# exoclime/HELIOS

Measured on AMD Instinct MI355X. Metric: rad-conv iterations/sec x (lambda-bins x layers), higher is better.
Workload: dtype f64; 1 GPU; BASELINE config 2: single column, 10 000 bins x 100 layers, premixed corr-k, isotropic scattering; nbin=10000, nlayer=100, ny=20, species=0, columns_per_gpu=1, columns_total=1, loop=radiative, parallelism=columns sharded, 1 per GPU

## Files before the change

helios_amd/csrc/rt_flux_kernel.inc:

```
template <int ROWS, int K = 0, bool MATRIX = false>
HX_FLUX_HEAD {
    using CT = HX_PLANE_T;
    extern __shared__ __align__(16) double smem[];
    const int col = a.reverse ? (int)(gridDim.y - 1 - blockIdx.y) : (int)blockIdx.y;
    if (a.done[col]) return;
    const int bx = a.reverse ? (int)(gridDim.x - 1 - blockIdx.x) : (int)blockIdx.x;
    const bool keep_state_cached = (int)(blockIdx.y * gridDim.x + blockIdx.x) >= a.cache_state_from;
    const int NN = a.H + 3, I = a.I;
    double* sB = smem;
    double* acc = sB + (size_t)a.nxb * NN;
    double* stage = acc + (size_t)a.nxb * 2 * I;
    const hx_rt_column cp = a.colpar[col];
    const size_t nc = (size_t)a.Y * a.X;
    const int k = K ? K : a.k;

    for (int t = threadIdx.x; t < a.nxb * NN; t += blockDim.x) {
        const int xl = t / NN, n = t - xl * NN, x = bx * a.nxb + xl;
        sB[t] = x < a.X ? a.Bn[((size_t)col * a.X + x) * NN + n] : 0.0;
    }
    for (int t = threadIdx.x; t < a.nxb * 2 * I; t += blockDim.x) acc[t] = 0.0;
    __syncthreads();

    for (int part = 0; part < a.nparts; part++) {
        const LaneMap m = lane_map(a, bx, part, opaque_tid());
        const size_t toff = m.tile * (size_t)ROWS * 64 + m.lane;
        const CT* ctile = HX_PLANES + col * a.coef_col + m.tile * (size_t)a.nplane * ROWS * 64 + m.lane;
        double* utile = a.Utile + col * a.flux_col + toff;
        double al[ROWS], be[ROWS], sd[ROWS], su[ROWS], Uo[ROWS], Do[ROWS];
#pragma unroll
        for (int r = 0; r < ROWS; r++) {
            al[r] = __builtin_nontemporal_load(ctile + (0 * ROWS + r) * 64);
            be[r] = __builtin_nontemporal_load(ctile + (1 * ROWS + r) * 64);
            sd[r] = __builtin_nontemporal_load(ctile + (2 * ROWS + r) * 64);
            if (!MATRIX) Uo[r] = __builtin_nontemporal_load(utile + r * 64);
        }
        if constexpr (sizeof(CT) == sizeof(double)) {
            if (a.has_vp) {
#pragma unroll
                for (int r = 0; r < ROWS; r++) su[r] = __builtin_nontemporal_load(ctile + (a.pl_vp * ROWS + r) * 64);
            } else {
#pragma unroll
                for (int r = 0; r < ROWS; r++) su[r] = a.Kconst * ((1.0 - al[r]) - be[r]) - sd[r];
            }
        } else {
            if (a.has_vp) {
#pragma unroll
                for (int r = 0; r < ROWS; r++) su[r] = __builtin_nontemporal_load(ctile + (a.pl_vp * ROWS + r) * 64);
            }
#pragma unroll
            for (int r = 0; r < ROWS; r++) {
                const double rest = plane_decode(al[r], be[r]);
                su[r] = (a.has_vp ? su[r] : a.Kconst * rest) - sd[r];
            }
        }
        double U0 = 0.0, boaK = 0.0, Fdir0 = 0.0, albedo = 0.0;
        if (m.valid && m.j == 0) {
            if (!MATRIX) U0 = a.U0[col * nc + m.sp];
            boaK = a.boaK[col * nc + m.sp];
            Fdir0 = a.Fdir0[col * nc + m.sp];
            albedo = a.surf_albedo[(size_t)col * a.X + m.x];
        }
        const double w = m.valid ? 0.5 * a.gauss_w[m.y] : 0.0;
        const double* Bx = sB + (size_t)(m.valid ? m.xl : 0) * NN;
#pragma unroll
        for (int r = 0; r < ROWS; r++) {
            const int h = min(m.j * ROWS + r, a.H - 1);
            const double Bb = Bx[h], Bt = a.iso ? Bb : Bx[h + 1], upc = sd[r], vpc = su[r];
            sd[r] = upc * Bb + vpc * Bt;
            su[r] = upc * Bt + vpc * Bb;
        }
        if (a.dir_beam == 1) {
            constexpr int BEAM_GROUP = ROWS <= 8 ? ROWS : HX_BEAM_GROUP;
#pragma unroll
            for (int r0 = 0; r0 < ROWS; r0 += BEAM_GROUP) {
                double bd[BEAM_GROUP], bu[BEAM_GROUP];
#pragma unroll
                for (int u = 0; u < BEAM_GROUP; u++)
                    if (r0 + u < ROWS) {
                        bd[u] = __builtin_nontemporal_load(ctile + (a.pl_dd * ROWS + r0 + u) * 64);
                        bu[u] = __builtin_nontemporal_load(ctile + ((a.pl_dd + 1) * ROWS + r0 + u) * 64);
                    }
                __builtin_amdgcn_sched_barrier(0);
#pragma unroll
                for (int u = 0; u < BEAM_GROUP; u++)
                    if (r0 + u < ROWS) {
                        sd[r0 + u] += bd[u];
                        su[r0 + u] += bu[u];
                    }
                __builtin_amdgcn_sched_barrier(0);
            }
        }
        const double rs = cp.R_star / cp.a;
        const double D_toa = (1.0 - a.dir_beam) * cp.f_factor * (rs * rs) * HX_PI * Bx[a.H + 1];
        const double B_surf = Bx[a.H + 2];

        const bool odd0 = (m.j * ROWS) & 1;
        const double thr_even = (a.iso || odd0) ? 1e-100 : 0.0, thr_odd = (a.iso || !odd0) ? 1e-100 : 0.0;
        if constexpr (MATRIX) {
            const bool scatters = m.valid ? a.trigger[col * nc + m.sp] != 0 : false;
            const bool flip_negative = scatters && !a.iso;
            const double tiny_d = scatters ? 0.0 : 1e-100;
            const double tiny_u_even = scatters ? 0.0 : ((a.iso || odd0) ? 1e-100 : 0.0), tiny_u_odd = scatters ? 0.0 : ((a.iso || !odd0) ? 1e-100 : 0.0);
            auto patch = [&](double v, double tiny) { return flip_negative ? (v < 1e-100 ? fabs(v) : v) : tiny_abs_below(v, tiny); };
            Moebius P = {1.0, 0.0, 0.0, 1.0};
#pragma unroll
            for (int r = 0; r < ROWS; r++) {
                const double omb = 1.0 - be[r];
                const double m11 = fma(al[r], al[r], be[r] * omb), m12 = (omb - al[r]) * (omb + al[r]);
                const double n11 = fma(m11, P.p11, m12 * P.p21), n12 = fma(m11, P.p12, m12 * P.p22);
                P.p21 = fma(be[r], P.p11, omb * P.p21);
                P.p22 = fma(be[r], P.p12, omb * P.p22);
                P.p11 = n11;
                P.p12 = n12;
            }
            {
                const double sc = 1.0 / fmax(fmax(fabs(P.p11), fabs(P.p12)), fmax(fabs(P.p21), fabs(P.p22)));
                P.p11 *= sc; P.p12 *= sc; P.p21 *= sc; P.p22 *= sc;
            }
            moebius_scan_up<K>(P, m.j, k);
            double e11 = K ? below_fixed<K>(P.p11) : from_lane_below<1>(P.p11, k), e12 = K ? below_fixed<K>(P.p12) : from_lane_below<1>(P.p12, k);
            double e21 = K ? below_fixed<K>(P.p21) : from_lane_below<1>(P.p21, k), e22 = K ? below_fixed<K>(P.p22) : from_lane_below<1>(P.p22, k);
            const double alb = K ? group_first_lane<K>(albedo, m.lane) : __shfl(albedo, 0, k);
            double rho = 1.0 - fma(e11, 1.0 - alb, e12) / fma(e21, 1.0 - alb, e22);
            if (m.j == 0) rho = alb;
#pragma unroll
            for (int r = 0; r < ROWS; r++) {
                const double inv = HX_MATRIX_RCP(1.0 - be[r] * rho), aa = al[r] * inv;
                su[r] = fma(aa * rho, sd[r], su[r]);
                rho = fma(aa * al[r], rho, be[r]);
                Uo[r] = rho;
                be[r] *= inv;
                sd[r] *= inv;
                al[r] = aa;
            }
            double sigma0 = 0.0;
            if (m.j == 0) sigma0 = albedo * Fdir0 + (1.0 - albedo) * HX_PI * boaK * B_surf;
            sigma0 = K ? group_first_lane<K>(sigma0, m.lane) : __shfl(sigma0, 0, k);
            {
                double A = 1.0, Bc = 0.0;
#pragma unroll
                for (int r = 0; r < ROWS; r++) {
                    Bc = fma(al[r], Bc, su[r]);
                    A *= al[r];
                }
                if (K) {
                    scan_up_fixed<K>(A, Bc, m.j);
                } else if (k == 32) {
                    scan32_up(A, Bc, m.j);
                } else {
                    scan_step_up<1>(A, Bc, m.j, k);
                    scan_step_up<2>(A, Bc, m.j, k);
                    scan_step_up<4>(A, Bc, m.j, k);
                    scan_step_up<8>(A, Bc, m.j, k);
                    scan_step_up<16>(A, Bc, m.j, k);
                    scan_step_up<32>(A, Bc, m.j, k);
                }
                double sg = K ? below_fixed<K>(fma(A, sigma0, Bc)) : from_lane_below<1>(fma(A, sigma0, Bc), k);
                if (m.j == 0) sg = sigma0;
#pragma unroll
                for (int r = 0; r < ROWS; r++) {
                    sd[r] = fma(be[r], sg, sd[r]);
                    sg = fma(al[r], sg, su[r]);
                    su[r] = sg;
                }
            }
            {
                double A = 1.0, Bc = 0.0;
#pragma unroll
                for (int r = ROWS - 1; r >= 0; r--) {
                    Bc = fma(al[r], Bc, sd[r]);
                    A *= al[r];
                }
                if (K) {
                    scan_down_fixed<K>(A, Bc, m.j, m.lane);
                } else if (k == 32) {
                    scan32_down(A, Bc, m.j, m.lane);
                } else {
                    scan_step_down<1>(A, Bc, m.j, k);
                    scan_step_down<2>(A, Bc, m.j, k);
                    scan_step_down<4>(A, Bc, m.j, k);
                    scan_step_down<8>(A, Bc, m.j, k);
                    scan_step_down<16>(A, Bc, m.j, k);
                    scan_step_down<32>(A, Bc, m.j, k);
                }
                double D = K ? above_fixed<K>(fma(A, D_toa, Bc)) : from_lane_above<1>(fma(A, D_toa, Bc), k);
                if (m.j == k - 1) D = D_toa;
#pragma unroll
                for (int r = ROWS - 1; r >= 0; r--) {
                    Uo[r] = patch(fma(Uo[r], D, su[r]), (r & 1) ? tiny_u_odd : tiny_u_even);
                    D = patch(fma(al[r], D, sd[r]), tiny_d);
                    Do[r] = D;
                }
            }
            if (m.j == 0) U0 = patch(fma(albedo, Do[0], sigma0), 0.0);
        } else
        for (int sweep = 0; sweep < a.nsweep; sweep++) {
            {
                double Ubelow = K ? below_fixed<K>(Uo[ROWS - 1]) : from_lane_below<1>(Uo[ROWS - 1], k);
                if (m.j == 0) Ubelow = U0;
                double A = 1.0, Bc = 0.0;
#pragma unroll
                for (int r = ROWS - 1; r >= 0; r--) {
                    const double Uh = r > 0 ? Uo[r - 1] : Ubelow;
                    const double t = fma(be[r], Uh, sd[r]);
                    Bc = fma(al[r], Bc, t);
                    A *= al[r];
                }
                if (K) {
                    scan_down_fixed<K>(A, Bc, m.j, m.lane);
                } else if (k == 32) {
                    scan32_down(A, Bc, m.j, m.lane);
                } else {
                    scan_step_down<1>(A, Bc, m.j, k);
                    scan_step_down<2>(A, Bc, m.j, k);
                    scan_step_down<4>(A, Bc, m.j, k);
                    scan_step_down<8>(A, Bc, m.j, k);
                    scan_step_down<16>(A, Bc, m.j, k);
                    scan_step_down<32>(A, Bc, m.j, k);
                }
                double Din = K ? above_fixed<K>(fma(A, D_toa, Bc)) : from_lane_above<1>(fma(A, D_toa, Bc), k);
                if (m.j == k - 1) Din = D_toa;
                double D = Din;
#pragma unroll
                for (int r = ROWS - 1; r >= 0; r--) {
                    const double Uh = r > 0 ? Uo[r - 1] : Ubelow;
                    D = tiny_abs(fma(al[r], D, fma(be[r], Uh, sd[r])));
                    Do[r] = D;
                }
            }
            if (m.j == 0) U0 = albedo * (Fdir0 + Do[0]) + (1.0 - albedo) * HX_PI * boaK * B_surf;
            const double Ubc = K ? group_first_lane<K>(U0, m.lane) : __shfl(U0, 0, k);
            {
                double Dabove = K ? above_fixed<K>(Do[0]) : from_lane_above<1>(Do[0], k);
                if (m.j == k - 1) Dabove = D_toa;
                double A = 1.0, Bc = 0.0;
#pragma unroll
                for (int r = 0; r < ROWS; r++) {
                    const double Dh = r < ROWS - 1 ? Do[r + 1] : Dabove;
                    const double t = fma(be[r], Dh, su[r]);
                    Bc = fma(al[r], Bc, t);
                    A *= al[r];
                }
                if (K) {
                    scan_up_fixed<K>(A, Bc, m.j);
                } else if (k == 32) {
                    scan32_up(A, Bc, m.j);
                } else {
                    scan_step_up<1>(A, Bc, m.j, k);
                    scan_step_up<2>(A, Bc, m.j, k);
                    scan_step_up<4>(A, Bc, m.j, k);
                    scan_step_up<8>(A, Bc, m.j, k);
                    scan_step_up<16>(A, Bc, m.j, k);
                    scan_step_up<32>(A, Bc, m.j, k);
                }
                double Uin = K ? below_fixed<K>(fma(A, Ubc, Bc)) : from_lane_below<1>(fma(A, Ubc, Bc), k);
                if (m.j == 0) Uin = Ubc;
                double U = Uin;
#pragma unroll
                for (int r = 0; r < ROWS; r++) {
                    const double Dh = r < ROWS - 1 ? Do[r + 1] : Dabove;
                    U = fma(al[r], U, fma(be[r], Dh, su[r]));
                    if (K) U = tiny_abs_below(U, (r & 1) ? thr_odd : thr_even);
                    else if (a.iso || ((m.j * ROWS + r) & 1)) U = tiny_abs(U);
                    Uo[r] = U;
                }
            }
        }

        const LaneMap e = lane_map(a, bx, part, opaque_tid());
#ifdef HX_PROFILING
        const int debug_skip = a.debug_skip;
#else
        constexpr int debug_skip = 0;
#endif
        auto store_state = [&]() {
            const size_t eoff = e.tile * (size_t)ROWS * 64 + e.lane;
            if (!(debug_skip & 2) && (!MATRIX || a.keep_up)) {
                double* ut = a.Utile + col * a.flux_col + eoff;
#pragma unroll
                for (int r = 0; r < ROWS; r++) {
                    if (keep_state_cached) __hip_atomic_store(ut + r * 64, Uo[r], __ATOMIC_RELAXED, __HIP_MEMORY_SCOPE_AGENT);
                    else __builtin_nontemporal_store(Uo[r], ut + r * 64);
                }
            }
            if (a.keep_down) {
                double* dtile = a.Dtile + col * a.flux_col + eoff;
#pragma unroll
                for (int r = 0; r < ROWS; r++) __builtin_nontemporal_store(Do[r], dtile + r * 64);
            }
            if (e.valid && e.j == 0) a.U0[col * nc + e.sp] = U0;
        };
        if (!(debug_skip & 1)) {
            if (e.valid) {
                const int h0 = e.j * ROWS, nrow = a.H - h0;
                double* st = stage + ((size_t)e.yl * a.nxb + e.xl) * 2 * I;
                if (a.iso) {
                    double *pd = st + h0, *pu = st + I + h0 + 1;
#pragma unroll
                    for (int r = 0; r < ROWS; r++)
                        if (r < nrow) {
                            pd[r] = w * Do[r];
                            pu[r] = w * Uo[r];
                        }
                } else {
                    const bool p = h0 & 1;
                    const int q = (h0 + (p ? 1 : 0)) >> 1;
                    double* pe = st + q + (p ? I : 0);
                    double* po = st + q + (p ? -1 : I);
#pragma unroll
                    for (int r = 0; r < ROWS; r++)
                        if (r < nrow) {
                            if ((r & 1) == 0) pe[r >> 1] = w * (p ? Uo[r] : Do[r]);
                            else po[(r + 1) >> 1] = w * (p ? Do[r] : Uo[r]);
                        }
                }
                if (e.j == 0) st[I + 0] = w * U0;
                if (h0 <= a.H - 1 && a.H - 1 < h0 + ROWS) st[a.L] = w * D_toa;
            }
            __syncthreads();
            for (int t = threadIdx.x; t < a.nxb * 2 * I; t += blockDim.x) {
                const int xl = t / (2 * I), rest = t - xl * 2 * I;
                double s = acc[t];
                for (int yl = 0; yl < a.ypb; yl++) s += stage[((size_t)yl * a.nxb + xl) * 2 * I + rest];
                acc[t] = s;
            }
            __syncthreads();
        }
        store_state();
    }
    for (int t = threadIdx.x; t < a.nxb * 2 * I; t += blockDim.x) {
        const int xl = t / (2 * I), rest = t - xl * 2 * I, x = bx * a.nxb + xl;
        if (x >= a.X) continue;
        const int dir = rest / I, i = rest - dir * I;
        (dir == 0 ? a.F_down_band_n : a.F_up_band_n)[((size_t)col * a.X + x) * I + i] = acc[t];
    }
}
```

helios_amd/csrc/rt_kernels.h:

```cpp
#pragma once
#include "rt_fused.h"
#include "conv_adjust.h"
#include "temp_step.h"
#include "two_stream.h"
#include "plane_code.h"

namespace hx {

struct KArgs {
    int X, Y, L, I, H, C;
    int k, ROWS, S, nxb, ypb, nparts, G, NW, nblk_x, nblk, nplane, nchunk, coef_nbx;
    int cloud_lds;
    int scat, dir_beam, clouds, scat_corr, nsweep, keep_down, real_star;
    int iso;
    int has_vp, pl_vp, pl_dd;
    int matrix;
    int* trigger;
    double Kconst;
    int dim, step;
    double epsi, epsi2, g_0, i2s, w_0_limit, w_0_scat_limit, dtau_limit;
    const hx_rt_column* colpar;
    const double *T_lay, *p_lay, *p_int, *dcol_u, *dcol_l, *surf_albedo, *Bstar, *planck_grid;
    const double *opac_wg_lay, *opac_wg_int, *scat_cross_lay, *scat_cross_int, *mmm_lay, *mmm_int;
    const double *cl_abs_lay, *cl_abs_int, *cl_sc_lay, *cl_sc_int, *g0_tot_lay, *g0_tot_int;
    double *half_ray, *half_g0, *half_cab, *half_csc;
    const double *F_dir_wg, *Fc_dir_wg, *F_dir_band_n, *gauss_w, *deltawave;
    double *T_int, *Bn, *coef, *Utile, *Dtile, *U0, *boaK, *Fdir0;
    double *dtau_u, *dtau_l;
    double *F_down_band_n, *F_up_band_n, *tot_part, *F_up_tot, *F_down_tot, *F_net;
    size_t coef_col, flux_col;
    const int* done;
    const TableSet* coltab;
    const double *ktemp, *kpress;
    const TPIndex *tp_lay, *tp_int;
    int ntemp, npress, from_table;
    unsigned long long* diag;
    int* iter_dev;
};

struct FluxArgs {
    int X, Y, L, I, H;
    int k, nxb, ypb, nparts, G, NW;
    int dir_beam, nsweep, keep_down, has_vp, pl_vp, pl_dd, nplane, iso, debug_skip;
    int keep_up;
    int reverse;
    int cache_state_from;
    const int* trigger;
    double Kconst;
    const hx_rt_column* colpar;
    const double *Bn, *coef, *U0_in, *boaK, *Fdir0, *surf_albedo, *gauss_w;
    double *Utile, *Dtile, *U0, *F_down_band_n, *F_up_band_n;
    size_t coef_col, flux_col;
    const int* done;
};

__device__ __forceinline__ double interface_T(const double* T, int i, int L) {
    if (i == 0) return T[0] - 0.5 * (T[1] - T[0]);
    if (i == L) return T[L - 1] + 0.5 * (T[L - 1] - T[L - 2]);
    return T[i - 1] + 0.5 * (T[i] - T[i - 1]);
}

__host__ __device__ __forceinline__ size_t plane_off(int r, int lane, int ROWS) {
    (void)ROWS;
    return (size_t)r * 64 + lane;
}

#ifndef HX_PLANE_KERNELS_ONLY
__global__ void __launch_bounds__(256) k_rt_nodes(KArgs a) {
    __shared__ double tile[32][33];
    const int col = blockIdx.z;
    if (blockIdx.x == 0 && blockIdx.y == 0 && blockIdx.z == 0 && threadIdx.x == 0 && a.iter_dev != nullptr) {
        const int cur = a.iter_dev[0];
        a.iter_dev[1] = cur;
        a.iter_dev[0] = cur + 1;
    }
    if (a.done[col]) return;
    const int NN = a.H + 3;
    const double* T = a.T_lay + (size_t)col * (a.L + 1);
    const int x0 = blockIdx.x * 32, n0 = blockIdx.y * 32;
    const int tx = threadIdx.x & 31, ty = threadIdx.x >> 5;
    if (blockIdx.x == 0 && blockIdx.y == 0)
        for (int i = threadIdx.x; i < a.I; i += blockDim.x)
            a.T_int[(size_t)col * a.I + i] = interface_T(T, i, a.L);
    enum { DEAD, STAR, LEVEL, INT_BOTTOM, INT_TOP, INT_MID };
    const int x = x0 + tx, xc = min(x, a.X - 1);
    int kind[4];
    double Ta[4], Tb[4], star[4];
#pragma unroll
    for (int q = 0; q < 4; q++) {
        const int n = n0 + ty + 8 * q, i = n >> 1;
        int kd, ia, ib = 0;
        if (!(n < NN && x < a.X)) { kd = DEAD; ia = 0; }
        else if (n == a.H + 1) { kd = STAR; ia = 0; }
        else if (n == a.H + 2) { kd = LEVEL; ia = a.L; }
        else if (a.iso) { kd = LEVEL; ia = min(n, a.L - 1); }
        else if (n & 1) { kd = LEVEL; ia = (n - 1) >> 1; }
        else if (i == 0) { kd = INT_BOTTOM; ia = 0; ib = 1; }
        else if (i == a.L) { kd = INT_TOP; ia = a.L - 1; ib = max(a.L - 2, 0); }
        else { kd = INT_MID; ia = i - 1; ib = i; }
        kind[q] = kd;
        Ta[q] = T[ia];
        Tb[q] = T[ib];
        star[q] = kd == STAR ? a.Bstar[(size_t)col * a.X + x] : 0.0;
    }
    int tdown[4], tup[4];
    double tt[4], gd[4], gu[4];
#pragma unroll
    for (int q = 0; q < 4; q++) {
        double Tn = Ta[q];
        if (kind[q] == INT_BOTTOM) Tn = Ta[q] - 0.5 * (Tb[q] - Ta[q]);
        else if (kind[q] == INT_TOP) Tn = Ta[q] + 0.5 * (Ta[q] - Tb[q]);
        else if (kind[q] == INT_MID) Tn = Ta[q] + 0.5 * (Tb[q] - Ta[q]);
        double t = (Tn - 1.0) / a.step;
        t = dmax(0.001, dmin(a.dim - 1.001, t));
        tt[q] = t;
        tdown[q] = (int)floor(t);
        tup[q] = (int)ceil(t);
        gd[q] = a.planck_grid[xc + (size_t)tdown[q] * a.X];
        gu[q] = a.planck_grid[xc + (size_t)tup[q] * a.X];
    }
#pragma unroll
    for (int q = 0; q < 4; q++) {
        double v = gd[q];
        if (tdown[q] != tup[q]) v = gd[q] * (tup[q] - tt[q]) + gu[q] * (tt[q] - tdown[q]);
        if (kind[q] == STAR) v = star[q];
        if (kind[q] != DEAD) tile[ty + 8 * q][tx] = v;
    }
    __syncthreads();
    for (int r = ty; r < 32; r += 8) {
        const int x = x0 + r, n = n0 + tx;
        if (n < NN && x < a.X) a.Bn[((size_t)col * a.X + x) * NN + n] = tile[tx][r];
    }
}

#endif
template <int CTRL, int ROW_MASK>
__device__ __forceinline__ double dpp_move(double v) {
    int lo = __double2loint(v), hi = __double2hiint(v);
    lo = __builtin_amdgcn_update_dpp(lo, lo, CTRL, ROW_MASK, 0xf, false);
    hi = __builtin_amdgcn_update_dpp(hi, hi, CTRL, ROW_MASK, 0xf, false);
    return __hiloint2double(hi, lo);
}

template <int N>
__device__ __forceinline__ double from_lane_below(double v, int k) {
    if (N == 1 && k == 32) return dpp_move<0x138, 0xf>(v);
    if (N < 16 && k <= 16) {
        int lo = __double2loint(v), hi = __double2hiint(v);
        lo = __builtin_amdgcn_update_dpp(lo, lo, 0x110 + (N & 15), 0xf, 0xf, false);
        hi = __builtin_amdgcn_update_dpp(hi, hi, 0x110 + (N & 15), 0xf, 0xf, false);
        return __hiloint2double(hi, lo);
    } else {
        return __shfl_up(v, N);
    }
}
template <int N>
__device__ __forceinline__ double from_lane_above(double v, int k) {
    if (N == 1 && k == 32) return dpp_move<0x130, 0xf>(v);
    if (N < 16 && k <= 16) {
        int lo = __double2loint(v), hi = __double2hiint(v);
        lo = __builtin_amdgcn_update_dpp(lo, lo, 0x100 + (N & 15), 0xf, 0xf, false);
        hi = __builtin_amdgcn_update_dpp(hi, hi, 0x100 + (N & 15), 0xf, 0xf, false);
        return __hiloint2double(hi, lo);
    } else {
        return __shfl_down(v, N);
    }
}

template <int N>
__device__ __forceinline__ void scan_step_down(double& A, double& Bc, int j, int k) {
    if (N < k) {
        const double A2 = from_lane_above<N>(A, k), B2 = from_lane_above<N>(Bc, k);
        if (j + N < k) {
            Bc = fma(A, B2, Bc);
            A *= A2;
        }
    }
}
template <int N>
__device__ __forceinline__ void scan_step_up(double& A, double& Bc, int j, int k) {
    if (N < k) {
        const double A2 = from_lane_below<N>(A, k), B2 = from_lane_below<N>(Bc, k);
        if (j >= N) {
            Bc = fma(A, B2, Bc);
            A *= A2;
        }
    }
}

__device__ __forceinline__ double group_lane16(double v, int lane) {
    const int lo = __double2loint(v), hi = __double2hiint(v);
    const int lo_a = __builtin_amdgcn_readlane(lo, 16), lo_b = __builtin_amdgcn_readlane(lo, 48);
    const int hi_a = __builtin_amdgcn_readlane(hi, 16), hi_b = __builtin_amdgcn_readlane(hi, 48);
    return __hiloint2double(lane < 32 ? hi_a : hi_b, lane < 32 ? lo_a : lo_b);
}

#define HX_SCAN32_ROW_STEP(CTRL, COND)                                              \
    {                                                                               \
        const double A2 = dpp_move<CTRL, 0xf>(A), B2 = dpp_move<CTRL, 0xf>(Bc);     \
        if (COND) {                                                                 \
            Bc = fma(A, B2, Bc);                                                    \
            A *= A2;                                                                \
        }                                                                           \
    }

__device__ __forceinline__ void scan32_down(double& A, double& Bc, int j, int lane) {
    const int jr = j & 15;
    HX_SCAN32_ROW_STEP(0x101, jr + 1 < 16)
    HX_SCAN32_ROW_STEP(0x102, jr + 2 < 16)
    HX_SCAN32_ROW_STEP(0x104, jr + 4 < 16)
    HX_SCAN32_ROW_STEP(0x108, jr + 8 < 16)
    const double A2 = group_lane16(A, lane), B2 = group_lane16(Bc, lane);
    if (j < 16) {
        Bc = fma(A, B2, Bc);
        A *= A2;
    }
}

__device__ __forceinline__ void scan32_up(double& A, double& Bc, int j) {
    const int jr = j & 15;
    HX_SCAN32_ROW_STEP(0x111, jr >= 1)
    HX_SCAN32_ROW_STEP(0x112, jr >= 2)
    HX_SCAN32_ROW_STEP(0x114, jr >= 4)
    HX_SCAN32_ROW_STEP(0x118, jr >= 8)
    const double A2 = dpp_move<0x142, 0xa>(A), B2 = dpp_move<0x142, 0xa>(Bc);
    if (j >= 16) {
        Bc = fma(A, B2, Bc);
        A *= A2;
    }
}
#undef HX_SCAN32_ROW_STEP

struct LaneMap {
    int lane, wv, j, x, y, xl, yl;
    bool valid;
    size_t sp;
    size_t tile;
};

__device__ __forceinline__ int opaque_tid() {
    int t = threadIdx.x;
    asm volatile("" : "+v"(t));
    return t;
}

template <class Args>
__device__ __forceinline__ LaneMap lane_map(const Args& a, int bx, int part, int tid) {
    LaneMap m;
    m.lane = tid & 63;
    m.wv = tid >> 6;
    m.j = m.lane & (a.k - 1);
    const int s_local = tid >> (31 - __clz(a.k));
    m.xl = s_local / a.ypb;
    m.yl = s_local - m.xl * a.ypb;
    m.x = bx * a.nxb + m.xl;
    m.y = part * a.ypb + m.yl;
    m.valid = s_local < a.G && m.x < a.X;
    m.sp = (size_t)m.y + (size_t)a.Y * m.x;
    m.tile = ((size_t)bx * a.nparts + part) * a.NW + m.wv;
    return m;
}

template <int CTRL>
__device__ __forceinline__ void compose_row_neighbour(double& A, double& Bc) {
    const int a_lo = __builtin_amdgcn_update_dpp(0, __double2loint(A), CTRL, 0xf, 0xf, true);
    const int a_hi = __builtin_amdgcn_update_dpp(0x3FF00000, __double2hiint(A), CTRL, 0xf, 0xf, false);
    const int b_lo = __builtin_amdgcn_update_dpp(0, __double2loint(Bc), CTRL, 0xf, 0xf, true);
    const int b_hi = __builtin_amdgcn_update_dpp(0, __double2hiint(Bc), CTRL, 0xf, 0xf, true);
    Bc = fma(A, __hiloint2double(b_hi, b_lo), Bc);
    A *= __hiloint2double(a_hi, a_lo);
}

template <int CTRL>
__device__ __forceinline__ double dpp_or_zero(double v) {
    const int lo = __builtin_amdgcn_update_dpp(0, __double2loint(v), CTRL, 0xf, 0xf, true);
    const int hi = __builtin_amdgcn_update_dpp(0, __double2hiint(v), CTRL, 0xf, 0xf, true);
    return __hiloint2double(hi, lo);
}

template <int SRC>
__device__ __forceinline__ double wave_lane(double v) {
    return __hiloint2double(__builtin_amdgcn_readlane(__double2hiint(v), SRC), __builtin_amdgcn_readlane(__double2loint(v), SRC));
}

template <int K>
__device__ __forceinline__ void scan_down_fixed(double& A, double& Bc, int j, int lane) {
    compose_row_neighbour<0x101>(A, Bc);
    compose_row_neighbour<0x102>(A, Bc);
    compose_row_neighbour<0x104>(A, Bc);
    compose_row_neighbour<0x108>(A, Bc);
    if (K == 32 || K == 64) {
        const double A2 = group_lane16(A, lane), B2 = group_lane16(Bc, lane);
        if ((lane & 16) == 0) {
            Bc = fma(A, B2, Bc);
            A *= A2;
        }
    }
    if (K == 64) {
        const double A2 = wave_lane<32>(A), B2 = wave_lane<32>(Bc);
        if (lane < 32) {
            Bc = fma(A, B2, Bc);
            A *= A2;
        }
    }
}
template <int K>
__device__ __forceinline__ void scan_up_fixed(double& A, double& Bc, int j) {
    compose_row_neighbour<0x111>(A, Bc);
    compose_row_neighbour<0x112>(A, Bc);
    compose_row_neighbour<0x114>(A, Bc);
    compose_row_neighbour<0x118>(A, Bc);
    if (K == 32 || K == 64) {
        const double A2 = dpp_move<0x142, 0xa>(A), B2 = dpp_move<0x142, 0xa>(Bc);
        if (j & 16) {
            Bc = fma(A, B2, Bc);
            A *= A2;
        }
    }
    if (K == 64) {
        const double A2 = dpp_move<0x143, 0xc>(A), B2 = dpp_move<0x143, 0xc>(Bc);
        if (j >= 32) {
            Bc = fma(A, B2, Bc);
            A *= A2;
        }
    }
}
template <int K>
__device__ __forceinline__ double below_fixed(double v) {
    return K == 16 ? dpp_or_zero<0x111>(v) : dpp_or_zero<0x138>(v);
}
template <int K>
__device__ __forceinline__ double above_fixed(double v) {
    return K == 16 ? dpp_or_zero<0x101>(v) : dpp_or_zero<0x130>(v);
}
template <int K>
__device__ __forceinline__ double group_first_lane(double v, int lane) {
    if (K == 16) return dpp_or_zero<0x150>(v);
    if (K == 64) return wave_lane<0>(v);
    const int lo = __double2loint(v), hi = __double2hiint(v);
    const int lo_a = __builtin_amdgcn_readlane(lo, 0), lo_b = __builtin_amdgcn_readlane(lo, 32);
    const int hi_a = __builtin_amdgcn_readlane(hi, 0), hi_b = __builtin_amdgcn_readlane(hi, 32);
    return __hiloint2double(lane < 32 ? hi_a : hi_b, lane < 32 ? lo_a : lo_b);
}
__device__ __forceinline__ double tiny_abs_below(double F, double thr) { return fabs(F) < thr ? fabs(F) : F; }

#ifndef HX_PLANE_KERNELS_ONLY
__global__ void __launch_bounds__(256) k_rt_half_bands(KArgs a) {
    __shared__ double tile[4][32][33];
    const int col = blockIdx.z;
    if (a.done[col]) return;
    const int tx = threadIdx.x & 31, ty = threadIdx.x >> 5;
    const size_t bandI = (size_t)a.X * a.I;
    const double* src_i[4] = {a.scat_cross_int + col * bandI, a.g0_tot_int + col * bandI, a.cl_abs_int + col * bandI,
                              a.cl_sc_int + col * bandI};
    const double* src_l[4] = {a.scat_cross_lay + col * bandI, a.g0_tot_lay + col * bandI, a.cl_abs_lay + col * bandI,
                              a.cl_sc_lay + col * bandI};
    double* dst[4] = {a.half_ray, a.half_g0, a.half_cab, a.half_csc};
    const int nq = a.clouds == 1 ? 4 : 1;
    const int x = blockIdx.x * 32 + tx;
    for (int hh = ty; hh < 32; hh += 8) {
        const int h = blockIdx.y * 32 + hh;
        if (x < a.X && h < a.H) {
            const int i = a.iso ? h : h >> 1, ii = a.iso ? h : i + (h & 1);
            const size_t b_l = x + (size_t)a.X * i, b_i = x + (size_t)a.X * ii;
            for (int q = 0; q < nq; q++) {
                const bool on = q == 1 || q == 2 || a.scat == 1;
                tile[q][hh][tx] = !on ? 0.0 : a.iso ? src_l[q][b_l] : (src_i[q][b_i] + src_l[q][b_l]) / 2.0;
            }
        }
    }
    __syncthreads();
    const int h = blockIdx.y * 32 + tx;
    for (int xx = ty; xx < 32; xx += 8) {
        const int xo = blockIdx.x * 32 + xx;
        if (xo < a.X && h < a.H)
            for (int q = 0; q < nq; q++) dst[q][((size_t)col * a.X + xo) * a.H + h] = tile[q][tx][xx];
    }
}

#endif

#define HX_COEF_KERNEL k_rt_coef
#define HX_PLANE_T double
#define HX_PLANE_ARG
#define HX_PLANES a.coef
#include "rt_coef_kernel.inc"
#undef HX_COEF_KERNEL
#undef HX_PLANE_T
#undef HX_PLANE_ARG
#undef HX_PLANES
#define HX_COEF_KERNEL k_rt_coef_f32
#define HX_PLANE_T float
#define HX_PLANE_ARG , float* coef32
#define HX_PLANES coef32
#include "rt_coef_kernel.inc"
#undef HX_COEF_KERNEL
#undef HX_PLANE_T
#undef HX_PLANE_ARG
#undef HX_PLANES
struct CoefPlainFlags {
    static constexpr int matrix = 0, iso = 0, dir_beam = 0, clouds = 0, cloud_lds = 0, scat_corr = 0, has_vp = 0;
    static constexpr double g_0 = 0.0;
    static constexpr unsigned long long* diag = nullptr;
};
#define HX_COEF_KERNEL k_rt_coef_plain
#define HX_PLANE_T double
#define HX_PLANE_ARG
#define HX_PLANES a.coef
#define HX_COEF_FLAG(name) CoefPlainFlags::name
#define HX_COEF_FROM_TABLE FROM_TABLE
#define HX_COEF_TEMPLATE template <int ROWS, int COEF_TPB, bool FROM_TABLE>
#include "rt_coef_kernel.inc"
#undef HX_COEF_KERNEL
#undef HX_PLANE_T
#undef HX_PLANE_ARG
#undef HX_PLANES
#undef HX_COEF_FLAG
#undef HX_COEF_FROM_TABLE
#undef HX_COEF_TEMPLATE

#ifndef HX_PLANE_KERNELS_ONLY
__global__ void __launch_bounds__(256) k_rt_dtau_halves(KArgs a) {
    const int col = blockIdx.z, i = blockIdx.y;
    const size_t nc = (size_t)a.Y * a.X;
    const size_t c = (size_t)blockIdx.x * blockDim.x + threadIdx.x;
    if (c >= nc || a.done[col]) return;
    const int x = (int)(c / a.Y);
    const size_t wgI = nc * a.I, bandI = (size_t)a.X * a.I;
    const double* opl = a.opac_wg_lay + col * wgI;
    const double* opi = a.opac_wg_int + col * wgI;
    const double* scl = a.scat_cross_lay + col * bandI;
    const double* sci = a.scat_cross_int + col * bandI;
    const double* mml = a.mmm_lay + (size_t)col * a.I;
    const double* mmi = a.mmm_int + (size_t)col * a.I;
    const size_t b = x + (size_t)a.X * i, k = c + nc * i;
    if (a.iso) {
        const double* pint = a.p_int + (size_t)col * a.I;
        const double ray = a.scat == 1 ? scl[b] : 0.0;
        a.dtau_u[col * nc * a.L + k] = (pint[i] - pint[i + 1]) / a.colpar[col].g * (opl[k] + ray / mml[i]);
        return;
    }
    double ray_up = 0, ray_low = 0;
    if (a.scat == 1) {
        ray_up = (scl[b] + sci[b + a.X]) / 2.0;
        ray_low = (sci[b] + scl[b]) / 2.0;
    }
    const double kap_up = (opl[k] + opi[k + nc]) / 2.0, kap_low = (opi[k] + opl[k]) / 2.0;
    const double mu_up = (mml[i] + mmi[i + 1]) / 2.0, mu_low = (mmi[i] + mml[i]) / 2.0;
    const size_t wgL = nc * a.L;
    a.dtau_u[col * wgL + k] = a.dcol_u[(size_t)col * a.L + i] * (kap_up + ray_up / mu_up);
    a.dtau_l[col * wgL + k] = a.dcol_l[(size_t)col * a.L + i] * (kap_low + ray_low / mu_low);
}
#endif

#ifndef HX_MATRIX_RCP
#define HX_MATRIX_RCP(x) newton_rcp(x)
#endif
__device__ __forceinline__ double newton_rcp(double x) {
    double r = __builtin_amdgcn_rcp(x);
    r = fma(fma(-x, r, 1.0), r, r);
    r = fma(fma(-x, r, 1.0), r, r);
    return r;
}

struct Moebius {
    double p11, p12, p21, p22;
};
__device__ __forceinline__ void moebius_after(Moebius& P, double q11, double q12, double q21, double q22) {
    const double n11 = fma(P.p11, q11, P.p12 * q21), n12 = fma(P.p11, q12, P.p12 * q22);
    const double n21 = fma(P.p21, q11, P.p22 * q21), n22 = fma(P.p21, q12, P.p22 * q22);
    P.p11 = n11; P.p12 = n12; P.p21 = n21; P.p22 = n22;
}
template <int CTRL, bool ONE>
__device__ __forceinline__ double dpp_or_identity(double v) {
    const int lo = __builtin_amdgcn_update_dpp(0, __double2loint(v), CTRL, 0xf, 0xf, true);
    const int hi = ONE ? __builtin_amdgcn_update_dpp(0x3FF00000, __double2hiint(v), CTRL, 0xf, 0xf, false)
                       : __builtin_amdgcn_update_dpp(0, __double2hiint(v), CTRL, 0xf, 0xf, true);
    return __hiloint2double(hi, lo);
}
template <int CTRL>
__device__ __forceinline__ void moebius_row_neighbour(Moebius& P) {
    moebius_after(P, dpp_or_identity<CTRL, true>(P.p11), dpp_or_identity<CTRL, false>(P.p12), dpp_or_identity<CTRL, false>(P.p21),
                  dpp_or_identity<CTRL, true>(P.p22));
}
template <int K>
__device__ __forceinline__ void moebius_scan_up(Moebius& P, int j, int k) {
    if (K) {
        moebius_row_neighbour<0x111>(P);
        moebius_row_neighbour<0x112>(P);
        moebius_row_neighbour<0x114>(P);
        moebius_row_neighbour<0x118>(P);
        if (K == 32 || K == 64) {
            const double q11 = dpp_move<0x142, 0xa>(P.p11), q12 = dpp_move<0x142, 0xa>(P.p12), q21 = dpp_move<0x142, 0xa>(P.p21),
                         q22 = dpp_move<0x142, 0xa>(P.p22);
            if (j & 16) moebius_after(P, q11, q12, q21, q22);
        }
        if (K == 64) {
            const double q11 = dpp_move<0x143, 0xc>(P.p11), q12 = dpp_move<0x143, 0xc>(P.p12), q21 = dpp_move<0x143, 0xc>(P.p21),
                         q22 = dpp_move<0x143, 0xc>(P.p22);
            if (j >= 32) moebius_after(P, q11, q12, q21, q22);
        }
    } else {
#define HX_MOEBIUS_STEP(N)                                                                                              \
    if (N < k) {                                                                                                        \
        const double q11 = from_lane_below<N>(P.p11, k), q12 = from_lane_below<N>(P.p12, k),                            \
                     q21 = from_lane_below<N>(P.p21, k), q22 = from_lane_below<N>(P.p22, k);                            \
        if (j >= N) moebius_after(P, q11, q12, q21, q22);                                                               \
    }
        HX_MOEBIUS_STEP(1) HX_MOEBIUS_STEP(2) HX_MOEBIUS_STEP(4) HX_MOEBIUS_STEP(8) HX_MOEBIUS_STEP(16) HX_MOEBIUS_STEP(32)
#undef HX_MOEBIUS_STEP
    }
}

#ifndef HX_BEAM_GROUP
#define HX_BEAM_GROUP 4
#endif
#ifndef HX_BIG_ROWS_ONE_WAVE
#define HX_BIG_ROWS_ONE_WAVE 1
#endif
constexpr bool flux_one_wave(int rows) { return rows >= 15 && HX_BIG_ROWS_ONE_WAVE; }
#define HX_FLUX_HEAD __global__ void __launch_bounds__(flux_one_wave(ROWS) ? 64 : 320) k_rt_flux(FluxArgs a)
#define HX_PLANE_T double
#define HX_PLANES a.coef
#include "rt_flux_kernel.inc"
#undef HX_FLUX_HEAD
#undef HX_PLANE_T
#undef HX_PLANES
#define HX_FLUX_HEAD __device__ __forceinline__ void rt_flux_f32_body(FluxArgs a, const float* coef32)
#define HX_PLANE_T float
#define HX_PLANES coef32
#include "rt_flux_kernel.inc"
#undef HX_FLUX_HEAD
#undef HX_PLANE_T
#undef HX_PLANES
template <int ROWS, int K = 0, bool MATRIX = false>
__global__ void __launch_bounds__(flux_one_wave(ROWS) ? 64 : 320) k_rt_flux_f32(FluxArgs a, const float* coef32) {
    rt_flux_f32_body<ROWS, K, MATRIX>(a, coef32);
}

#ifndef HX_PLANE_KERNELS_ONLY
__global__ void __launch_bounds__(256) __attribute__((amdgpu_waves_per_eu(1, 2))) k_rt_totals_a(KArgs a) {
    const int col = blockIdx.y, chunk = blockIdx.x;
    if (a.done[col]) return;
    const int I = a.I;
    const int per = (a.X + a.nchunk - 1) / a.nchunk;
    const int x0 = chunk * per, x1 = min(a.X, x0 + per);
    const double* __restrict__ fdir = a.F_dir_band_n + (size_t)col * a.X * I;
    const double* __restrict__ dl = a.deltawave;
    for (int t = threadIdx.x; t < 2 * I; t += blockDim.x) {
        const int dir = t / I, i = t - dir * I;
        const double* __restrict__ band = (dir == 0 ? a.F_down_band_n : a.F_up_band_n) + (size_t)col * a.X * I;
        constexpr int NB = 24;
        double acc = 0.0;
        for (int xb = x0; xb < x1; xb += NB) {
            double v[NB], w[NB];
#pragma unroll
            for (int u = 0; u < NB; u++) {
                const int x = min(xb + u, x1 - 1);
                const unsigned o = (unsigned)x * (unsigned)I + (unsigned)i;
                const double f = fdir[o], b = band[o];
                v[u] = dir == 0 ? f + b : b;
                w[u] = dl[x];
            }
#pragma unroll
            for (int u = 0; u < NB; u++)
                if (xb + u < x1) acc += v[u] * w[u];
        }
        a.tot_part[(((size_t)col * a.nchunk + chunk) * 2) * I + t] = acc;
    }
}

struct TotalsBArgs {
    KArgs a;
    RadTempArgs rt;
    int step_temperature;
    int* done_w;
    int* iters_done;
    const int* iter_dev;
    size_t sL, sL1, sI;
};

__global__ void __launch_bounds__(1024) k_rt_totals_b(TotalsBArgs q) {
    const KArgs& a = q.a;
    const int col = blockIdx.x;
    if (a.done[col]) return;
    const int I = a.I, L = a.L;
    double* up = a.F_up_tot + (size_t)col * I;
    double* down = a.F_down_tot + (size_t)col * I;
    double* net = a.F_net + (size_t)col * I;
    __shared__ double seg[4][256];
    for (int t0 = 0; t0 < 2 * I; t0 += 256) {
        const int t = t0 + (threadIdx.x & 255), sgm = threadIdx.x >> 8;
        const int cper = (a.nchunk + 3) / 4, c0 = sgm * cper, c1 = min(a.nchunk, c0 + cper);
        double s = 0.0;
        if (t < 2 * I) {
            const double* __restrict__ part = a.tot_part + ((size_t)col * a.nchunk * 2) * I + t;
            for (int cb = c0; cb < c1; cb += 8) {
                double v[8];
#pragma unroll
                for (int u = 0; u < 8; u++) v[u] = part[(size_t)min(cb + u, c1 - 1) * 2 * I];
#pragma unroll
                for (int u = 0; u < 8; u++)
                    if (cb + u < c1) s += v[u];
            }
        }
        seg[sgm][threadIdx.x & 255] = s;
        __syncthreads();
        if (sgm == 0 && t < 2 * I) {
            const double tot = ((seg[0][threadIdx.x] + seg[1][threadIdx.x]) + seg[2][threadIdx.x]) + seg[3][threadIdx.x];
            if (t < I) down[t] = tot; else up[t - I] = tot;
        }
        __syncthreads();
    }
    for (int i = threadIdx.x; i < I; i += blockDim.x) net[i] = up[i] - down[i];
    __syncthreads();
    if (!q.step_temperature) return;
    const hx_rt_column cp = a.colpar[col];
    const int itervalue = q.iter_dev != nullptr ? q.iter_dev[1] : q.rt.itervalue;
    if (itervalue < cp.foreplay) return;
    RadTempArgs r = q.rt;
    r.itervalue = itervalue;
    r.F_down_tot = down;
    r.F_net = net;
    r.F_net_diff += (size_t)col * L;
    r.tlay += (size_t)col * (L + 1);
    r.play += (size_t)col * L;
    r.pint += (size_t)col * I;
    r.abrt += (size_t)col * (L + 1);
    r.T_store += (size_t)col * (L + 1);
    r.deltat_prefactor += (size_t)col * (L + 1);
    r.F_add_heat_lay += (size_t)col * L;
    r.F_add_heat_sum += (size_t)col * L;
    r.F_smooth += (size_t)col * L;
    r.F_smooth_sum += (size_t)col * L;
    r.c_p_lay += (size_t)col * L;
    r.meanmolmass_lay = a.mmm_lay + (size_t)col * I;
    r.conv_count += col;
    r.foreplay = cp.foreplay;
    r.g = cp.g;
    r.physical_tstep = cp.physical_tstep;
    r.local_limit = cp.rad_convergence_limit;
    r.adapt_interval = cp.adapt_interval;
    r.F_intern = cp.F_intern;
    r.no_atmo = cp.no_atmo;
    rad_temp_step(r, threadIdx.x, blockDim.x);
    __syncthreads();
    if (threadIdx.x == 0 && *r.conv_count == L + 1) {
        q.done_w[col] = 1;
        q.iters_done[col] = r.itervalue + 1;
    }
}

struct ConvKArgs {
    int L, C, itervalue;
    const hx_rt_column* colpar;
    double* T_lay;
    const double *p_lay, *p_int;
    const double *kappa_lay, *kappa_int;
    const double *c_p, *mmm_lay;
    const double *F_add_heat_sum, *F_smooth_sum;
    const double *F_down_tot, *F_up_tot, *F_net;
    int *conv_unstable, *conv_layer, *marked_red;
    const double* dampara;
    const int* done;
};

__device__ __forceinline__ ConvColumn conv_column(const ConvKArgs& a, int col) {
    const size_t L = a.L, I = a.L + 1;
    const hx_rt_column cp = a.colpar[col];
    ConvColumn c;
    c.T = a.T_lay + col * I;
    c.p_lay = a.p_lay + col * L;
    c.p_int = a.p_int + col * I;
    c.kappa_lay = a.kappa_lay + col * L;
    c.kappa_int = a.kappa_int + col * I;
    c.c_p = a.c_p + col * L;
    c.mmm = a.mmm_lay + col * I;
    c.F_add_heat_sum = a.F_add_heat_sum + col * L;
    c.F_smooth_sum = a.F_smooth_sum + col * L;
    c.F_down_tot = a.F_down_tot + col * I;
    c.F_up_tot = a.F_up_tot + col * I;
    c.F_net = a.F_net + col * I;
    c.conv_unstable = a.conv_unstable + col * I;
    c.conv_layer = a.conv_layer + col * I;
    c.marked_red = a.marked_red + col * I;
    c.L = a.L;
    c.itervalue = a.itervalue;
    c.F_intern = cp.F_intern;
    c.T_star = cp.T_star;
    c.dampara = a.dampara[col];
    c.rad_convergence_limit = cp.rad_convergence_limit;
    return c;
}

__global__ void __launch_bounds__(256) k_rt_conv_adjust(ConvKArgs a) {
    extern __shared__ __align__(16) double conv_smem[];
    __shared__ ConvTables t;
    const int col = blockIdx.x;
    if (a.done[col]) return;
    __shared__ ConvShared sh;
    ConvColumn c = conv_column(a, col), g;
    conv_stage_in(c, g, t, conv_smem, threadIdx.x, blockDim.x);
    convective_adjustment_wg(c, t, sh, threadIdx.x, blockDim.x);
    conv_stage_out(c, g, threadIdx.x, blockDim.x);
}

struct TotalsCArgs {
    KArgs a;
    ConvKArgs cv;
    ConvTempArgs ct;
    int* done_w;
    int* iters_done;
    int physical_tstep_on;
};

__global__ void __launch_bounds__(1024) k_rt_totals_c(TotalsCArgs q) {
    extern __shared__ __align__(16) double conv_smem[];
    __shared__ ConvTables t;
    __shared__ double seg[4][256];
    __shared__ int s_go;
    const KArgs& a = q.a;
    const int col = blockIdx.x;
    if (a.done[col]) return;
    const int I = a.I, L = a.L;
    double* up = a.F_up_tot + (size_t)col * I;
    double* down = a.F_down_tot + (size_t)col * I;
    double* net = a.F_net + (size_t)col * I;
    for (int t0 = 0; t0 < 2 * I; t0 += 256) {
        const int ts = t0 + (threadIdx.x & 255), sgm = threadIdx.x >> 8;
        const int cper = (a.nchunk + 3) / 4, c0 = sgm * cper, c1 = min(a.nchunk, c0 + cper);
        double s = 0.0;
        if (ts < 2 * I) {
            const double* __restrict__ part = a.tot_part + ((size_t)col * a.nchunk * 2) * I + ts;
            for (int cb = c0; cb < c1; cb += 8) {
                double v[8];
#pragma unroll
                for (int u = 0; u < 8; u++) v[u] = part[(size_t)min(cb + u, c1 - 1) * 2 * I];
#pragma unroll
                for (int u = 0; u < 8; u++)
                    if (cb + u < c1) s += v[u];
            }
        }
        seg[sgm][threadIdx.x & 255] = s;
        __syncthreads();
        if (sgm == 0 && ts < 2 * I) {
            const double tot = ((seg[0][threadIdx.x] + seg[1][threadIdx.x]) + seg[2][threadIdx.x]) + seg[3][threadIdx.x];
            if (ts < I) down[ts] = tot; else up[ts - I] = tot;
        }
        __syncthreads();
    }
    for (int i = threadIdx.x; i < I; i += blockDim.x) net[i] = up[i] - down[i];
    __syncthreads();
    ConvColumn c = conv_column(q.cv, col), g;
    conv_stage_in(c, g, t, conv_smem, threadIdx.x, blockDim.x);
    __shared__ ConvShared sh;
    __shared__ int s_convective;
    conv_find_lim(c, sh, threadIdx.x, blockDim.x);
    conv_mark_layers_wg(c, t, sh, 1, threadIdx.x, blockDim.x);
    int go = 0;
    if (!q.physical_tstep_on) {
        const int eq = conv_radiative_eq_wg(c, sh, &s_convective, threadIdx.x, blockDim.x);
        go = (!eq) || (c.itervalue < 400) || (s_convective == 0);
    }
    if (threadIdx.x == 0) {
        if (!go) {
            q.done_w[col] = 1;
            q.iters_done[col] = c.itervalue;
        }
        s_go = go;
    }
    __syncthreads();
    conv_stage_out(c, g, threadIdx.x, blockDim.x);
    __syncthreads();
    if (!s_go) return;
    const hx_rt_column cp = a.colpar[col];
    ConvTempArgs r = q.ct;
    r.F_net = net;
    r.F_net_diff += (size_t)col * L;
    r.tlay += (size_t)col * (L + 1);
    r.play += (size_t)col * L;
    r.pint += (size_t)col * I;
    r.T_store += (size_t)col * (L + 1);
    r.deltat_prefactor += (size_t)col * (L + 1);
    r.marked_red = g.marked_red;
    r.F_add_heat_lay += (size_t)col * L;
    r.F_smooth += (size_t)col * L;
    r.F_smooth_sum += (size_t)col * L;
    r.adapt_interval = cp.adapt_interval;
    r.F_intern = cp.F_intern;
    conv_temp_step(r, threadIdx.x, blockDim.x);
}

__global__ void k_rt_tint(const double* __restrict__ T_lay, double* __restrict__ T_int, int L, const int* done) {
    const int col = blockIdx.y, i = blockIdx.x * blockDim.x + threadIdx.x;
    if (i > L || done[col]) return;
    T_int[(size_t)col * (L + 1) + i] = interface_T(T_lay + (size_t)col * (L + 1), i, L);
}

__global__ void k_rt_heating(const double* __restrict__ dens, const double* __restrict__ dz,
                             double* __restrict__ F_lay, double* __restrict__ F_sum, int L, const int* done) {
    const int col = blockIdx.x;
    if (threadIdx.x != 0 || done[col]) return;
    dens += (size_t)col * L; dz += (size_t)col * L; F_lay += (size_t)col * L; F_sum += (size_t)col * L;
    double run = 0.0;
    for (int i = 0; i < L; i++) {
        const double f = dens[i] * dz[i];
        F_lay[i] = f;
        run = i == 0 ? f : run + f;
        F_sum[i] = run;
    }
}

__global__ void k_rt_height(const double* __restrict__ p_lay, const double* __restrict__ dz,
                            double* __restrict__ z, int L, int gas, size_t stride, const int* __restrict__ done) {
    const int col = blockIdx.x;
    p_lay += col * stride; dz += col * stride; z += col * stride;
    if (threadIdx.x != 0 || done[col]) return;
    if (gas) {
        int i0 = 0;
        for (int i = 0; i < L; i++) if (p_lay[i] >= 1e7) i0 = i;
        z[i0] = 0.0;
        for (int i = i0 + 1; i < L; i++) z[i] = z[i - 1] + 0.5 * dz[i - 1] + 0.5 * dz[i];
        for (int i = i0 - 1; i >= 0; i--) z[i] = z[i + 1] - 0.5 * dz[i + 1] - 0.5 * dz[i];
    } else {
        z[0] = 0.5 * dz[0];
        for (int i = 1; i < L; i++) z[i] = z[i - 1] + 0.5 * dz[i - 1] + 0.5 * dz[i];
    }
}

__global__ void k_rt_meanmolmass(const double* __restrict__ vmr, const double* __restrict__ weight,
                                 const int* __restrict__ in_mu, double* __restrict__ out, int nspecies,
                                 int nlev) {
    const int i = blockIdx.x * blockDim.x + threadIdx.x;
    if (i >= nlev) return;
    double num = 0.0, tot = 0.0;
    for (int s = 0; s < nspecies; s++)
        if (in_mu[s]) {
            num += vmr[(size_t)s * nlev + i] * weight[s];
            tot += vmr[(size_t)s * nlev + i];
        }
    out[i] = num / tot * HX_AMU;
}

__global__ void __launch_bounds__(256) k_rt_fdir_band(const double* __restrict__ F_dir_wg,
                                                      double* __restrict__ out,
                                                      const double* __restrict__ gauss_w, int X, int Y,
                                                      int I, const int* __restrict__ done) {
    __shared__ double tile[32][33];
    const int col = blockIdx.z;
    if (done[col]) return;
    const int x0 = blockIdx.x * 32, i0 = blockIdx.y * 32, tx = threadIdx.x & 31, ty = threadIdx.x >> 5;
    F_dir_wg += (size_t)col * Y * X * I;
    out += (size_t)col * X * I;
    for (int lv = ty; lv < 32; lv += 8) {
        const int x = x0 + tx, i = i0 + lv;
        double s = 0.0;
        if (x < X && i < I) {
            const double* f = F_dir_wg + (size_t)Y * x + (size_t)Y * X * i;
            if (Y == 20) {
                double v[20];
#pragma unroll
                for (int y = 0; y < 20; y += 2) {
                    const double2 p = *(const double2*)(f + y);
                    v[y] = p.x;
                    v[y + 1] = p.y;
                }
#pragma unroll
                for (int y = 0; y < 20; y++) s += 0.5 * gauss_w[y] * v[y];
            } else {
                for (int y = 0; y < Y; y++) s += 0.5 * gauss_w[y] * f[y];
            }
        }
        tile[lv][tx] = s;
    }
    __syncthreads();
    for (int xx = ty; xx < 32; xx += 8) {
        const int x = x0 + xx, i = i0 + tx;
        if (x < X && i < I) out[(size_t)x * I + i] = tile[tx][xx];
    }
}

__global__ void k_rt_tp_index(TPLocate<true, false> src, TPIndex* tp_lay, TPIndex* tp_int, int L, int I, const int* done) {
    const int col = blockIdx.y, i = blockIdx.x * blockDim.x + threadIdx.x;
    if (i >= I || done[col]) return;
    tp_int[(size_t)col * I + i] = src.at(col, 1, i);
    if (i < L) tp_lay[(size_t)col * I + i] = src.at(col, 0, i);
}

__global__ void k_rt_delta_z(KArgs a, double* __restrict__ dz) {
    const int col = blockIdx.y, i = blockIdx.x * blockDim.x + threadIdx.x;
    if (i >= a.L || a.done[col]) return;
    const double* pint = a.p_int + (size_t)col * a.I;
    dz[(size_t)col * a.L + i] = HX_KBOLTZMANN * a.T_lay[(size_t)col * (a.L + 1) + i] /
                                (a.mmm_lay[(size_t)col * a.I + i] * a.colpar[col].g) * log(pint[i] / pint[i + 1]);
}

__global__ void __launch_bounds__(256) k_rt_total_g0(KArgs a, const double* __restrict__ g_cl_lay,
                                                     const double* __restrict__ g_cl_int, double* g_tot_lay,
                                                     double* g_tot_int) {
    const int col = blockIdx.z, lev = blockIdx.y;
    const int x = blockIdx.x * blockDim.x + threadIdx.x;
    if (x >= a.X || a.done[col]) return;
    const size_t k = (size_t)col * a.X * a.I + x + (size_t)a.X * lev;
    if (lev < a.L) {
        const double num = a.g_0 * a.scat_cross_lay[k] + g_cl_lay[k] * a.cl_sc_lay[k];
        g_tot_lay[k] = num / (a.scat_cross_lay[k] + a.cl_sc_lay[k]);
    }
    const double num = a.g_0 * a.scat_cross_int[k] + g_cl_int[k] * a.cl_sc_int[k];
    g_tot_int[k] = num / (a.scat_cross_int[k] + a.cl_sc_int[k]);
}

__global__ void k_rt_keep_ref_T(KArgs a, double* T_lay_ref, double* T_int_ref, TableSet* coltab_ref) {
    const int col = blockIdx.y, i = blockIdx.x * blockDim.x + threadIdx.x;
    if (a.done[col]) return;
    if (i == 0) coltab_ref[col] = a.coltab[col];
    if (i <= a.L) T_lay_ref[(size_t)col * (a.L + 1) + i] = a.T_lay[(size_t)col * (a.L + 1) + i];
    if (i < a.I) T_int_ref[(size_t)col * a.I + i] = a.T_int[(size_t)col * a.I + i];
}

__global__ void __launch_bounds__(256) k_rt_tile_rows(const double* __restrict__ src,
                                                      double* __restrict__ out, int X, int nlev) {
    const int x = blockIdx.x * blockDim.x + threadIdx.x, i = blockIdx.y;
    if (x < X) out[x + (size_t)X * i] = src[x];
}

#endif

}
```

Before: 2.620 billion bin*layer*iterations/s.

## Prefetch flux coefficient planes and state ahead of use in flux kernel

```diff
diff --git a/helios_amd/csrc/rt_flux_kernel.inc b/helios_amd/csrc/rt_flux_kernel.inc
--- a/helios_amd/csrc/rt_flux_kernel.inc
+++ b/helios_amd/csrc/rt_flux_kernel.inc
@@ -3,15 +3,50 @@
     using CT = HX_PLANE_T;
     extern __shared__ __align__(16) double smem[];
     const int col = a.reverse ? (int)(gridDim.y - 1 - blockIdx.y) : (int)blockIdx.y;
-    if (a.done[col]) return;
     const int bx = a.reverse ? (int)(gridDim.x - 1 - blockIdx.x) : (int)blockIdx.x;
+    const size_t nc = (size_t)a.Y * a.X;
+    constexpr bool REQUEST_HEAD = HX_FLUX_REQUEST_HEAD, REQUEST_AHEAD = HX_FLUX_REQUEST_AHEAD && flux_requests_ahead(ROWS);
+    CT ral[ROWS], rbe[ROWS], rsd[ROWS];
+    double Uo[ROWS];
+    double rU0 = 0.0, rboaK = 0.0, rFdir0 = 0.0, ralbedo = 0.0, rgw = 0.0;
+    auto request_planes = [&](int part) {
+        const LaneMap m = lane_map(a, bx, part, opaque_tid());
+        const CT* ctile = HX_PLANES + col * a.coef_col + m.tile * (size_t)a.nplane * ROWS * 64 + m.lane;
+#pragma unroll
+        for (int r = 0; r < ROWS; r++) {
+            ral[r] = __builtin_nontemporal_load(ctile + (0 * ROWS + r) * 64);
+            rbe[r] = __builtin_nontemporal_load(ctile + (1 * ROWS + r) * 64);
+            rsd[r] = __builtin_nontemporal_load(ctile + (2 * ROWS + r) * 64);
+        }
+        rU0 = 0.0, rboaK = 0.0, rFdir0 = 0.0, ralbedo = 0.0;
+        if (m.valid && m.j == 0) {
+            if (!MATRIX) rU0 = a.U0[col * nc + m.sp];
+            rboaK = a.boaK[col * nc + m.sp];
+            rFdir0 = a.Fdir0[col * nc + m.sp];
+            ralbedo = a.surf_albedo[(size_t)col * a.X + m.x];
+        }
+        rgw = m.valid ? a.gauss_w[m.y] : 0.0;
+    };
+    auto request_state = [&](int part) {
+        if (MATRIX) return;
+        const LaneMap m = lane_map(a, bx, part, opaque_tid());
+        const double* utile = a.Utile + col * a.flux_col + m.tile * (size_t)ROWS * 64 + m.lane;
+#pragma unroll
+        for (int r = 0; r < ROWS; r++) Uo[r] = __builtin_nontemporal_load(utile + r * 64);
+    };
+    const int done = a.done[col];
+    if (REQUEST_HEAD) {
+        request_planes(0);
+        request_state(0);
+        asm volatile("" ::: "memory");
+    }
+    if (done) return;
     const bool keep_state_cached = (int)(blockIdx.y * gridDim.x + blockIdx.x) >= a.cache_state_from;
     const int NN = a.H + 3, I = a.I;
     double* sB = smem;
     double* acc = sB + (size_t)a.nxb * NN;
     double* stage = acc + (size_t)a.nxb * 2 * I;
     const hx_rt_column cp = a.colpar[col];
-    const size_t nc = (size_t)a.Y * a.X;
     const int k = K ? K : a.k;
 
     for (int t = threadIdx.x; t < a.nxb * NN; t += blockDim.x) {
@@ -23,16 +58,20 @@
 
     for (int part = 0; part < a.nparts; part++) {
         const LaneMap m = lane_map(a, bx, part, opaque_tid());
-        const size_t toff = m.tile * (size_t)ROWS * 64 + m.lane;
+        if (part == 0 ? !REQUEST_HEAD : !REQUEST_AHEAD) {
+            request_planes(part);
+            request_state(part);
+        }
         const CT* ctile = HX_PLANES + col * a.coef_col + m.tile * (size_t)a.nplane * ROWS * 64 + m.lane;
-        double* utile = a.Utile + col * a.flux_col + toff;
-        double al[ROWS], be[ROWS], sd[ROWS], su[ROWS], Uo[ROWS], Do[ROWS];
+        double al[ROWS], be[ROWS], sd[ROWS], su[ROWS], Do[ROWS];
 #pragma unroll
         for (int r = 0; r < ROWS; r++) {
-            al[r] = __builtin_nontemporal_load(ctile + (0 * ROWS + r) * 64);
-            be[r] = __builtin_nontemporal_load(ctile + (1 * ROWS + r) * 64);
-            sd[r] = __builtin_nontemporal_load(ctile + (2 * ROWS + r) * 64);
-            if (!MATRIX) Uo[r] = __builtin_nontemporal_load(utile + r * 64);
+            al[r] = ral[r];
+            be[r] = rbe[r];
+            sd[r] = rsd[r];
+            ral[r] = __builtin_nondeterministic_value(ral[r]);
+            rbe[r] = __builtin_nondeterministic_value(rbe[r]);
+            rsd[r] = __builtin_nondeterministic_value(rsd[r]);
         }
         if constexpr (sizeof(CT) == sizeof(double)) {
             if (a.has_vp) {
@@ -53,14 +92,10 @@
                 su[r] = (a.has_vp ? su[r] : a.Kconst * rest) - sd[r];
             }
         }
-        double U0 = 0.0, boaK = 0.0, Fdir0 = 0.0, albedo = 0.0;
-        if (m.valid && m.j == 0) {
-            if (!MATRIX) U0 = a.U0[col * nc + m.sp];
-            boaK = a.boaK[col * nc + m.sp];
-            Fdir0 = a.Fdir0[col * nc + m.sp];
-            albedo = a.surf_albedo[(size_t)col * a.X + m.x];
-        }
-        const double w = m.valid ? 0.5 * a.gauss_w[m.y] : 0.0;
+        double U0 = rU0;
+        const double boaK = rboaK, Fdir0 = rFdir0, albedo = ralbedo;
+        double w = 0.5 * rgw;
+        asm volatile("" : "+v"(w));
         const double* Bx = sB + (size_t)(m.valid ? m.xl : 0) * NN;
 #pragma unroll
         for (int r = 0; r < ROWS; r++) {
@@ -265,6 +300,11 @@
                     Uo[r] = U;
                 }
             }
+        }
+
+        if (REQUEST_AHEAD && part + 1 < a.nparts) {
+            request_planes(part + 1);
+            __builtin_amdgcn_sched_barrier(0);
         }
 
         const LaneMap e = lane_map(a, bx, part, opaque_tid());
@@ -327,6 +367,7 @@
             __syncthreads();
         }
         store_state();
+        if (REQUEST_AHEAD && part + 1 < a.nparts) request_state(part + 1);
     }
     for (int t = threadIdx.x; t < a.nxb * 2 * I; t += blockDim.x) {
         const int xl = t / (2 * I), rest = t - xl * 2 * I, x = bx * a.nxb + xl;
diff --git a/helios_amd/csrc/rt_kernels.h b/helios_amd/csrc/rt_kernels.h
--- a/helios_amd/csrc/rt_kernels.h
+++ b/helios_amd/csrc/rt_kernels.h
@@ -519,6 +519,13 @@
 #define HX_BIG_ROWS_ONE_WAVE 1
 #endif
 constexpr bool flux_one_wave(int rows) { return rows >= 15 && HX_BIG_ROWS_ONE_WAVE; }
+#ifndef HX_FLUX_REQUEST_HEAD
+#define HX_FLUX_REQUEST_HEAD 1
+#endif
+#ifndef HX_FLUX_REQUEST_AHEAD
+#define HX_FLUX_REQUEST_AHEAD 1
+#endif
+constexpr bool flux_requests_ahead(int rows) { return true; }
 #define HX_FLUX_HEAD __global__ void __launch_bounds__(flux_one_wave(ROWS) ? 64 : 320) k_rt_flux(FluxArgs a)
 #define HX_PLANE_T double
 #define HX_PLANES a.coef
```

Result: no change. 2.640 billion bin*layer*iterations/s, median of 4 (+0.7%).
